# phlash/java-sdr

Hardware: AMD Instinct MI355X
Metric: IQ Msamples/s through FFT+FIR+BPSK demod, 2048-pt frames (higher is better)
Workload: dtype f64

## Files before the change

java-sdr_amd/csrc/bpsk_fm.hip:

```cpp
#include "bpsk_units.h"
#include "bpsk_tuner.h"
#include <math.h>
#include <type_traits>
#include <stddef.h>
#include <stdlib.h>

namespace jsdr {
namespace fm { __constant__ BpskConst c_bpsk; }
using fm::c_bpsk;
}
#include "bpsk_matched.h"

namespace jsdr {


template <bool FAST>
__global__ __launch_bounds__(512) void k_matched(MatchedArgs a)
{
    extern __shared__ __align__(16) unsigned char smem[];
    double2 *X = reinterpret_cast<double2 *>(smem);
    const int s = blockIdx.y;
    const long long G = a.tile0 + 4160LL * blockIdx.x;
    const double2 *dm = a.dm + (long long)s * a.dm_stride;
    {
// ... 69 lines not shown
__device__ unsigned long long g_fm_wgclk[WGCLK_SLOTS][WGCLK_WGS][3];
static long long g_wgclk_log[WGCLK_SLOTS][4];
#endif

__global__ void k_fm_edges(EdgeArgs a)
{
    const int t = blockIdx.x * blockDim.x + threadIdx.x;
    const int s = t / (4 * FM_EDGE), i = t % (4 * FM_EDGE);
    if (s >= a.nstreams) return;
    const int n = i < 2 * FM_EDGE ? i - FM_EDGE : a.nsamples - FM_EDGE + (i - 2 * FM_EDGE);
    int w = 0;
    if (n >= 0 && n < a.nsamples) {
        w = a.raw[(long long)s * a.stride_pairs + n];
    } else if (n < 0 && n >= -26) {
        w = a.hist[(long long)s * 32 + 26 + n].x;
        if (a.dc) {
            const int si = (int)(short)((w & 0xffff) - a.ic);
            const int sq = (int)(short)((w >> 16) - a.qc);
            w = (si & 0xffff) | (sq << 16);
        }
    }
    a.edges[(long long)s * (4 * FM_EDGE) + i] = w;
}

__global__ void k_fm_prep(EdgeArgs e, HistArgs hi, ScatterArgs sc)
{
    const int t = blockIdx.x * blockDim.x + threadIdx.x;
    const int nedge = e.nstreams * 4 * FM_EDGE;
    {
        const int v = t - nedge - 32 * e.nstreams;
        if (v >= 0) {
            if (v < sc.bytes[0]) sc.dst[0][v] = sc.src[0][v];
            else if (v - sc.bytes[0] < sc.bytes[1]) sc.dst[1][v - sc.bytes[0]] = sc.src[1][v - sc.bytes[0]];
            return;
        }
    }
    if (t < nedge) {
        const int s = t / (4 * FM_EDGE), i = t % (4 * FM_EDGE);
        const int n = i < 2 * FM_EDGE ? i - FM_EDGE : e.nsamples - FM_EDGE + (i - 2 * FM_EDGE);
        int w = 0;
        if (n >= 0 && n < e.nsamples) {
            w = e.raw[(long long)s * e.stride_pairs + n];
        } else if (n < 0 && n >= -26) {
            w = e.hist[(long long)s * 32 + 26 + n].x;
            if (e.dc) {
                const int si = (int)(short)((w & 0xffff) - e.ic);
                const int sq = (int)(short)((w >> 16) - e.qc);
                w = (si & 0xffff) | (sq << 16);
            }
        }
        e.edges[(long long)s * (4 * FM_EDGE) + i] = w;
        return;
    }
    const int u = t - nedge;
    const int s = u >> 5, i = u & 31;
    if (s >= hi.nstreams || i >= 26) return;
    const long long n = hi.nsamples - 26 + i;
    int2 v;
    if (n < 0) {
        v = hi.hist_old[(long long)s * 32 + (26 + n)];
    } else {
        const int w = hi.raw[(long long)s * hi.stride_pairs + n];
        const int si = java_short_add((int)(short)(w & 0xffff), hi.ic);
        const int sq = java_short_add(w >> 16, hi.qc);
        v = make_int2((si & 0xffff) | (sq << 16), 0);
    }
    hi.hist_new[(long long)s * 32 + i] = v;
}

constexpr bool ds_taps_are_short()
{
    for (int n = 0; n < 14; n++) {
        const float k = kDsHalf[n] * 32768.0f;
        if (k != (float)(int)k || k >= 16384.0f || k <= -16384.0f) return false;
    }
    return true;
}
static_assert(ds_taps_are_short(), "dsFilter: every tap times 2^15 is an integer of magnitude below 2^14 (k_fm's +-1.0 fmas are exact)");

template <int D, int R, bool MIX, bool DC, bool FAST, bool SMALL = false, int PH = -1>
#ifndef JSDR_FM_MINWAVES
#define JSDR_FM_MINWAVES 2
#endif
__global__ __launch_bounds__(FM_THREADS, JSDR_FM_MINWAVES) void k_fm(FmArgs a)
{
    constexpr int RD = D * R, NS = RD - D + 27, NSQ = (NS + 3) / 4;
    constexpr int JOBS = (FM_NT + R - 1) / R, ROUNDS = (JOBS + FM_THREADS - 1) / FM_THREADS;
    static_assert(PH < 0 || (MIX && !FAST && PH < 4 && (D * R) % 8 == 0 && (65 * FM_NB * D) % 8 == 4),
                  "k_fm<PH>: the lane span is whole periods and a tile is half a period past the one before");
    extern __shared__ __align__(16) unsigned char smem[];
    double2 *X = reinterpret_cast<double2 *>(smem);
    double *sc = reinterpret_cast<double *>(smem + FM_NT * sizeof(double2));
    for (int i = threadIdx.x; i < 512; i += FM_THREADS) sc[i] = a.sincos[i];
#ifdef JSDR_X_CLK
    unsigned long long clk_acc_[6] = {0, 0, 0, 0, 0, 0}, clk_last_ = 0;
#endif
#ifdef JSDR_X_WGCLK
    const unsigned long long wgclk0 = __builtin_amdgcn_s_memrealtime();
    unsigned long long wgclk_n = 0;
#endif
    const long long nwork = (long long)a.ntiles * a.nstreams;
    const bool tickets = a.tickets != nullptr;
    int *tkL = reinterpret_cast<int *>(sc + 512);
#pragma unroll 1
    for (long long work = blockIdx.x; work < nwork; work = tickets ? (long long)gridDim.x + (unsigned)__builtin_amdgcn_readfirstlane(tkL[0]) : work + gridDim.x) {
    const int s = (int)(work / a.ntiles);
    const long long G = a.tile0 + (long long)(65 * FM_NB) * (work % a.ntiles);
    const int jrel0 = (int)(G - 64 - a.g_first);
#ifdef JSDR_X_FM_SMALLSET
    const int *raw = a.raw + (long long)(s & 15) * a.stride_pairs;
#else
    const int *raw = a.raw + (long long)s * a.stride_pairs;
#endif
    const int *edges = a.edges + (long long)s * (4 * FM_EDGE);
    const double2 *dmh_old = a.dmh_old + (long long)s * 64;
    const int Lm1 = a.nsamples - 1, nds = a.nds, P = a.tper;
    const double HOWARD = 0.9 * 32768.0 * (double)I16_2P15_UNSCALE;
    int e0 = 0;
    if constexpr (MIX) {
        const long long v = (long long)a.first_out + (long long)D * jrel0;
        e0 = (int)(((v % P) + P) % P);
    }
    typedef const __attribute__((address_space(4))) double *const_tab_t;
    const_tab_t tb = (const_tab_t)(a.tcs + e0);
    float amx = 0.0f;
    __syncthreads();
#ifdef JSDR_X_CLK
    clk_last_ = __builtin_amdgcn_s_memtime();
#endif
    auto front = [&](auto phc) __attribute__((always_inline)) {
    constexpr int PHC = decltype(phc)::value;
#ifdef JSDR_X_NOFRONT
    if (a.nds < 0)
#endif
#pragma unroll 1
    for (int round = 0; round < ROUNDS; round++) {
        const int job = threadIdx.x + FM_THREADS * round;
        const int t0 = R * job;
        if (t0 >= FM_NT) break;
        const int j0 = jrel0 + t0;
        const int n0 = a.first_out + D * j0 - 26;
        const bool none = j0 + R <= 0 || j0 >= nds || nds <= 0;
        const bool regular = j0 >= 0 && j0 + R <= nds;
        if (!none) {
            int4 W[NSQ];
            const int *wp = raw + n0;
            if (n0 < 0) wp = edges + (n0 + FM_EDGE);
            else if (n0 + 4 * NSQ - 1 > Lm1) wp = edges + 2 * FM_EDGE + (n0 - (a.nsamples - FM_EDGE));
            unsigned kv4[(R + 3) / 4];
#pragma unroll
            for (int k = 0; k < (R + 3) / 4; k++) kv4[k] = 0;
            if (regular) {
#pragma unroll
                for (int r = 0; r < R; r++) kv4[r / 4] |= (unsigned)a.kvco[j0 + r] << (8 * (r % 4));
            } else {
#pragma unroll
                for (int r = 0; r < R; r++) {
                    const int j = j0 + r;
                    kv4[r / 4] |= (unsigned)a.kvco[j < 0 ? 0 : (j >= nds ? nds - 1 : j)] << (8 * (r % 4));
                }
            }
#pragma unroll
            for (int q = NSQ - 1; q >= 0; q--) W[q] = *reinterpret_cast<const int4 *>(wp + 4 * q);
#ifndef JSDR_FM_NOPIN
            __builtin_amdgcn_sched_barrier(0);
#endif
            double ai[R], aq[R];
            double vc[R], vs[R];
#pragma unroll
            for (int r = 0; r < R; r++) {
                ai[r] = 0.0;
                aq[r] = 0.0;
            }
#pragma unroll
            for (int q = NSQ - 1; q >= 0; q--) {
                const int4 w4 = W[q];
                if (q == 0) {
#pragma unroll
                    for (int r = 0; r < R; r++) {
                        const int kv = (kv4[r / 4] >> (8 * (r % 4))) & 0xff;
                        vc[r] = sc[kv];
                        vs[r] = sc[256 + kv];
                    }
                }
#pragma unroll
                for (int t = 3; t >= 0; t--) {
                    const int m = 4 * q + t;
                    if (m < NS) {
                        const int w = (t == 0) ? w4.x : (t == 1) ? w4.y : (t == 2) ? w4.z : w4.w;
                        double di, dq;
                        fm_convert_2p15(w, a.ic, a.qc, DC, di, dq, FAST ? &amx : nullptr);
                        const int ci = PHC >= 0 ? tuner8_class(PHC + m, 0) : TC_GEN, cq = PHC >= 0 ? tuner8_class(PHC + m, 1) : TC_GEN;
                        if constexpr (MIX) {
                            if (ci == TC_GEN) di = di * tb[2 * m];
                            if (cq == TC_GEN) dq = dq * tb[2 * m + 1];
                        }
#pragma unroll
                        for (int r = 0; r < R; r++) {
                            if (m >= D * r && m <= D * r + 26) {
                                const int age = D * r + 26 - m;
                                const double tp = ds_tap(age);
                                const bool same = age == 0 || ((kDsPow2Mask >> age) & 1);
                                if (FAST || same || ci != TC_GEN) {
                                    if (ci != TC_ZERO) ai[r] = __builtin_fma(di, ci == TC_MONE ? -tp : tp, ai[r]);
                                } else {
                                    ai[r] += di * tp;
                                }
                                if (FAST || same || cq != TC_GEN) {
                                    if (cq != TC_ZERO) aq[r] = __builtin_fma(dq, cq == TC_MONE ? -tp : tp, aq[r]);
                                } else {
                                    aq[r] += dq * tp;
                                }
                            }
                        }
                    }
                }
#ifndef JSDR_FM_NOPIN
#pragma unroll
                for (int r = 0; r < R; r++) asm volatile("" : "+v"(ai[r]), "+v"(aq[r])::"memory");
                if constexpr (FAST) asm volatile("" : "+v"(amx));
                __builtin_amdgcn_sched_barrier(0);
#endif
            }
            if (regular) {
#pragma unroll
                for (int r = 0; r < R; r++) {
                    const double oi = ai[r] * HOWARD, oq = aq[r] * HOWARD;
                    if (FM_NT % R == 0 || t0 + r < FM_NT) X[t0 + r] = make_double2(oi * vc[r], oq * vs[r]);
                }
            } else {
                double oi[R], oq[R];
#pragma unroll
                for (int r = 0; r < R; r++) {
                    oi[r] = ai[r] * HOWARD * vc[r];
                    oq[r] = aq[r] * HOWARD * vs[r];
                }
#pragma unroll 1
                for (int r = 0; r < R; r++) {
                    const int t = t0 + r, j = j0 + r;
                    double2 val = make_double2(0.0, 0.0);
                    if (j >= 0 && j < nds) {
                        val.x = r == 0 ? oi[0] : r == 1 ? oi[1] : r == 2 ? oi[2] : r == 3 ? oi[3] : oi[R - 1];
                        val.y = r == 0 ? oq[0] : r == 1 ? oq[1] : r == 2 ? oq[2] : r == 3 ? oq[3] : oq[R - 1];
                    } else if (j >= -64 && j < 0) {
                        val = dmh_old[64 + j];
                    }
                    if (t < FM_NT) X[t] = val;
                }
            }
        } else {
#pragma unroll 1
            for (int r = 0; r < R; r++) {
                const int t = t0 + r, j = j0 + r;
                const double2 val = (j >= -64 && j < 0) ? dmh_old[64 + j] : make_double2(0.0, 0.0);
                if (t < FM_NT) X[t] = val;
            }
        }
    }
    };
    if constexpr (PH < 0) {
        front(std::integral_constant<int, -1>{});
    } else {
        if (((e0 + a.trot) & 7) == PH) front(std::integral_constant<int, PH>{});
        else front(std::integral_constant<int, PH + 4>{});
    }
    if constexpr (FAST) {
#pragma unroll
        for (int off = 32; off >= 1; off >>= 1) amx = fmaxf(amx, __shfl_xor(amx, off, 64));
        if ((threadIdx.x & 63) == 0 && amx > 0.0f) atomicMax(a.amax + s, __float_as_int(amx));
    }
    FM_CLK(1);
    __syncthreads();
    FM_CLK(3);
    unsigned tk = 0;
    if (tickets && threadIdx.x == 0) tk = atomicAdd(a.tickets, 1u);
    if (jrel0 + FM_NT > nds - 64) {
        double2 *dmh_new = a.dmh_new + (long long)s * 64;
        for (int t = 64 + threadIdx.x; t < FM_NT; t += FM_THREADS) {
            const int j = jrel0 + t;
            if (j >= nds - 64 && j < nds && j >= 0) dmh_new[j - (nds - 64)] = X[t];
        }
        if (work % a.ntiles == 0 && nds < 64 && (int)threadIdx.x < 64 - nds) dmh_new[threadIdx.x] = dmh_old[threadIdx.x + nds];
    }
    const int lane = threadIdx.x & 63;
    const int wave = __builtin_amdgcn_readfirstlane(threadIdx.x >> 6);
    const int blk = lane < FM_NB ? lane : FM_NB - 1;
    const double2 *xl = X + 64 + 65 * blk;
    const int rel0 = jrel0 + 64 + 65 * blk;
    double2 *y = a.y + (long long)s * a.y_stride;
    if constexpr (SMALL) {
        const int rel = (int)threadIdx.x, t = rel - jrel0;
        if (rel < nds && t >= 64 && t < FM_NT) {
            const long long g = a.g_first + rel;
            const int u = (int)(((g - 64) % 65 + 65) % 65);
            const double2 *xg = X + t;
            const double *f = c_bpsk.dm_taps;
            double yi = 0.0, yq = 0.0;
            for (int i = 0; i <= 64 - u; i++) {
                const double2 x = xg[-(u + i)];
                const double tp = f[u + i];
                if constexpr (FAST) {
                    yi = __builtin_fma(x.x, tp, yi);
                    yq = __builtin_fma(x.y, tp, yq);
                } else {
                    yi += x.x * tp;
                    yq += x.y * tp;
                }
            }
            for (int m = 0; m < u; m++) {
                const double2 x = xg[-m];
                const double tp = f[m];
                if constexpr (FAST) {
                    yi = __builtin_fma(x.x, tp, yi);
                    yq = __builtin_fma(x.y, tp, yq);
                } else {
                    yi += x.x * tp;
                    yq += x.y * tp;
                }
            }
            y[rel] = make_double2(yi, yq);
        }
    } else {
#ifdef JSDR_X_NOMATCHED
    if (a.nds < 0)
#endif
#ifndef JSDR_FM_DIRECT_STORE
    {
        double ai[9], aq[9];
        int u0 = 0, nout = 9;
        if (wave == 0) {
            matched_block<9, FAST>(xl, 0, ai, aq);
        } else {
            u0 = 9 + 8 * (wave - 1);
            nout = 8;
            double bi[8], bq[8];
            matched_block<8, FAST>(xl, u0, bi, bq);
#pragma unroll
            for (int r = 0; r < 8; r++) {
                ai[r] = bi[r];
                aq[r] = bq[r];
            }
        }
        __syncthreads();
        if (lane < FM_NB) {
#pragma unroll
            for (int r = 0; r < 9; r++)
                if (r < nout) X[65 * blk + u0 + r] = make_double2(ai[r], aq[r]);
        }
        __syncthreads();
        const int relb = jrel0 + 64;
        for (int o = (int)threadIdx.x; o < 65 * FM_NB; o += FM_THREADS) {
            const int rel = relb + o;
            if (rel >= 0 && rel < nds) y[rel] = X[o];
        }
    }
#else
    if (wave == 0) {
        double ai[9], aq[9];
        matched_block<9, FAST>(xl, 0, ai, aq);
#pragma unroll
        for (int r = 0; r < 9; r++) {
            const int rel = rel0 + r;
            if (lane < FM_NB && rel >= 0 && rel < nds) y[rel] = make_double2(ai[r], aq[r]);
        }
    } else {
        const int u0 = 9 + 8 * (wave - 1);
        double ai[8], aq[8];
        matched_block<8, FAST>(xl, u0, ai, aq);
#pragma unroll
        for (int r = 0; r < 8; r++) {
            const int rel = rel0 + u0 + r;
            if (lane < FM_NB && rel >= 0 && rel < nds) y[rel] = make_double2(ai[r], aq[r]);
        }
    }
#endif
    }
    FM_CLK(4);
    {
        int zlate = 0;
        asm volatile("" : "+v"(zlate));
        if (tickets && threadIdx.x == 0) tkL[0] = (int)tk + zlate;
    }
    __syncthreads();
    FM_CLK(5);
#ifdef JSDR_X_WGCLK
    wgclk_n++;
#endif
    }
#ifdef JSDR_X_WGCLK
    if (threadIdx.x == 0 && blockIdx.x < WGCLK_WGS) {
        unsigned long long *c = g_fm_wgclk[a.wgclk_slot][blockIdx.x];
        c[0] = wgclk0;
        c[1] = __builtin_amdgcn_s_memrealtime();
        c[2] = wgclk_n;
    }
#endif
#ifdef JSDR_X_CLK
    if ((threadIdx.x & 63) == 0)
        for (int i = 0; i < 6; i++) atomicAdd(&g_fm_clk[blockIdx.x & 255][(threadIdx.x >> 6) * 8 + i], clk_acc_[i]);
#endif
}


int bpsk_fm_upload_constants(const BpskConst &bc)
{
    JSDR_HIP_TRY(hipMemcpyToSymbol(HIP_SYMBOL(c_bpsk), &bc, sizeof(bc)));
    return JSDR_OK;
}

int launch_matched(const MatchedArgs &ma, int nstreams, hipStream_t st)
{
    const long long ntiles = (ma.g_first + ma.nds - ma.tile0 + 4159) / 4160;
    const size_t lds = (64 + 4160) * sizeof(double2);
    JSDR_LDS_ATTR(k_matched<false>, lds);
    JSDR_LDS_ATTR(k_matched<true>, lds);
    hipLaunchKernelGGL(k_matched<false>, dim3((unsigned)ntiles, (unsigned)nstreams), dim3(512), lds, st, ma);
    return launched();
}

int launch_dm_history(double2 *dm, long long dm_stride, long long nds, int nstreams, hipStream_t st)
{
    hipLaunchKernelGGL(k_dm_history, dim3((unsigned)nstreams), dim3(64), 0, st, dm, dm_stride, nds, nstreams);
    return launched();
}

int launch_fm_prep(const EdgeArgs &ea, const HistArgs &ha, const ScatterArgs &sc, hipStream_t st)
{
    hipLaunchKernelGGL(k_fm_prep, dim3((unsigned)(((long long)ea.nstreams * (4 * FM_EDGE + 32) + sc.bytes[0] + sc.bytes[1] + 255) / 256)),
                       dim3(256), 0, st, ea, ha, sc);
    return launched();
}

template <int D, int R>
static int launch_fm_t(const FmArgs &a_in, bool mix, bool dc, bool fast, int nstreams, hipStream_t st, long long *items, long long *grid_out,
                       int *phase)
{
    *phase = -1;
    const size_t lds = (size_t)FM_NT * sizeof(double2) + 512 * sizeof(double) + sizeof(double);
    const long long span = 65LL * FM_NB;
    const long long ntiles = (a_in.g_first + a_in.nds - a_in.tile0 + span - 1) / span;
    FmArgs a = a_in;
    a.ntiles = (int)ntiles;
    a.nstreams = nstreams;
    static const long long grid_cap = [] {
        const char *e = knob("JSDR_FM_GRID");
        return e ? atoll(e) : 0LL;
    }();
    long long gx = ntiles * nstreams;
    if (grid_cap > 0 && gx > grid_cap) gx = grid_cap;
    if (a.grid_limit > 0 && gx > a.grid_limit) gx = a.grid_limit;
    *items = ntiles * nstreams;
    *grid_out = gx;
    if (!(a.grid_limit > 0 && gx < ntiles * nstreams && ntiles * nstreams + gx < 0x7fffffffLL)) a.tickets = nullptr;
#ifdef JSDR_X_WGCLK
    {
        static int wgclk_seq = 0;
        static const bool wgclk_static = getenv("JSDR_X_WGCLK_STATIC") != nullptr;
        if (wgclk_static) a.tickets = nullptr;
        a.wgclk_slot = wgclk_seq % WGCLK_SLOTS;
        g_wgclk_log[a.wgclk_slot][0] = ntiles * nstreams;
        g_wgclk_log[a.wgclk_slot][1] = gx;
        g_wgclk_log[a.wgclk_slot][2] = a.tickets != nullptr;
        g_wgclk_log[a.wgclk_slot][3] = wgclk_seq++;
    }
#endif
    if (a.tickets) JSDR_HIP_TRY(hipMemsetAsync(a.tickets, 0, sizeof(unsigned), st));
    const dim3 grid((unsigned)gx), block(FM_THREADS);
#define JSDR_FM_LAUNCH_PH(MIX, DC, FAST, SMALL, PH)                                                             \
    do {                                                                                                        \
        JSDR_LDS_ATTR((k_fm<D, R, MIX, DC, FAST, SMALL, PH>), lds);                                             \
        hipLaunchKernelGGL((k_fm<D, R, MIX, DC, FAST, SMALL, PH>), grid, block, lds, st, a);                    \
    } while (0)
#define JSDR_FM_LAUNCH(MIX, DC, FAST, SMALL) JSDR_FM_LAUNCH_PH(MIX, DC, FAST, SMALL, -1)
    const bool small = !fast && a.nds <= FM_THREADS && ntiles == 1;
    if constexpr (D == 10) {
        if (mix && !fast && !small && a.trot >= 0 && a.tper == 8) {
            const long long v = (long long)a.first_out + (long long)D * (a.tile0 - 64 - a.g_first);
            const int p0 = (int)((((v % 8) + 8) % 8 + a.trot) & 7);
            *phase = p0;
            switch (p0 & 3) {
                case 0: if (dc) JSDR_FM_LAUNCH_PH(true, true, false, false, 0); else JSDR_FM_LAUNCH_PH(true, false, false, false, 0); break;
                case 1: if (dc) JSDR_FM_LAUNCH_PH(true, true, false, false, 1); else JSDR_FM_LAUNCH_PH(true, false, false, false, 1); break;
                case 2: if (dc) JSDR_FM_LAUNCH_PH(true, true, false, false, 2); else JSDR_FM_LAUNCH_PH(true, false, false, false, 2); break;
                default: if (dc) JSDR_FM_LAUNCH_PH(true, true, false, false, 3); else JSDR_FM_LAUNCH_PH(true, false, false, false, 3); break;
// ... 76 lines not shown
```

java-sdr_amd/csrc/bpsk_fm_f32.hip:

```cpp
#include "bpsk_units.h"
#include <math.h>
#include <stddef.h>
#include <stdlib.h>

namespace jsdr {
namespace fm32 { __constant__ BpskConst c_bpsk; }
using fm32::c_bpsk;
}
#include "bpsk_matched.h"

namespace jsdr {

#ifndef JSDR_FM32_PQ
#define JSDR_FM32_PQ 6
#endif
enum { FM32_PQ = JSDR_FM32_PQ };

__global__ void k_fm_prep_f32(EdgeF32Args e, HistArgs hi)
{
    const int t = blockIdx.x * blockDim.x + threadIdx.x;
    const int nedge = e.nstreams * 4 * FM_EDGE;
    if (t < nedge) {
        const int s = t / (4 * FM_EDGE), i = t % (4 * FM_EDGE);
        const int n = i < 2 * FM_EDGE ? i - FM_EDGE : e.nsamples - FM_EDGE + (i - 2 * FM_EDGE);
        float2 w = make_float2(0.0f, 0.0f);
        if (n >= 0 && n < e.nsamples) {
            w = e.rawf[(long long)s * e.stride_pairs + n];
        } else if (n < 0 && n >= -26) {
            const int2 h = e.hist[(long long)s * 32 + 26 + n];
            w = make_float2(__int_as_float(h.x), __int_as_float(h.y));
        }
        e.edges[(long long)s * (4 * FM_EDGE) + i] = w;
        return;
    }
    const int u = t - nedge;
    const int s = u >> 5, i = u & 31;
    if (s >= hi.nstreams || i >= 26) return;
    const long long n = hi.nsamples - 26 + i;
    int2 v;
    if (n < 0) {
        v = hi.hist_old[(long long)s * 32 + (26 + n)];
    } else {
        const float2 f = hi.rawf[(long long)s * hi.stride_pairs + n];
        v = make_int2(__float_as_int(f.x), __float_as_int(f.y));
    }
    hi.hist_new[(long long)s * 32 + i] = v;
}

template <int D, int R, bool MIX, bool SMALL = false>
__global__ __launch_bounds__(FM_THREADS, 2) void k_fm_f32(FmF32Args fa)
{
    const FmArgs &a = fa.a;
    constexpr int RD = D * R, NS = RD - D + 27, NQ = (NS + 1) / 2;
    constexpr int PQ = FM32_PQ, NP = (NQ + PQ - 1) / PQ;
    constexpr int JOBS = (FM_NT + R - 1) / R, ROUNDS = (JOBS + FM_THREADS - 1) / FM_THREADS;
    static_assert(2 * NQ <= FM_EDGE, "a window must fit an edge image's half");
    extern __shared__ __align__(16) unsigned char smem[];
    double2 *X = reinterpret_cast<double2 *>(smem);
    double *sc = reinterpret_cast<double *>(smem + FM_NT * sizeof(double2));
    for (int i = threadIdx.x; i < 512; i += FM_THREADS) sc[i] = a.sincos[i];
    const long long nwork = (long long)a.ntiles * a.nstreams;
    const bool tickets = a.tickets != nullptr;
    int *tkL = reinterpret_cast<int *>(sc + 512);
#pragma unroll 1
    for (long long work = blockIdx.x; work < nwork; work = tickets ? (long long)gridDim.x + (unsigned)__builtin_amdgcn_readfirstlane(tkL[0]) : work + gridDim.x) {
    const int s = (int)(work / a.ntiles);
    const long long G = a.tile0 + (long long)(65 * FM_NB) * (work % a.ntiles);
    const int jrel0 = (int)(G - 64 - a.g_first);
    const float2 *raw = fa.rawf + (long long)s * a.stride_pairs;
    const float2 *edges = fa.edges + (long long)s * (4 * FM_EDGE);
    const double2 *dmh_old = a.dmh_old + (long long)s * 64;
    const int Lm1 = a.nsamples - 1, nds = a.nds, P = a.tper;
    const double HOWARD = 0.9 * 32768.0;
    int e0 = 0;
    if constexpr (MIX) {
        const long long v = (long long)a.first_out + (long long)D * jrel0;
        e0 = (int)(((v % P) + P) % P);
    }
    typedef const __attribute__((address_space(4))) double *const_tab_t;
    const_tab_t tb = (const_tab_t)(a.tcs + e0);
    __syncthreads();
#pragma unroll 1
    for (int round = 0; round < ROUNDS; round++) {
        const int job = threadIdx.x + FM_THREADS * round;
        const int t0 = R * job;
        if (t0 >= FM_NT) break;
        const int j0 = jrel0 + t0;
        const int n0 = a.first_out + D * j0 - 26;
        const bool none = j0 + R <= 0 || j0 >= nds || nds <= 0;
        const bool regular = j0 >= 0 && j0 + R <= nds;
        if (!none) {
            const float2 *wp = raw + n0;
            if (n0 < 0) wp = edges + (n0 + FM_EDGE);
            else if (n0 + 2 * NQ - 1 > Lm1) wp = edges + 2 * FM_EDGE + (n0 - (a.nsamples - FM_EDGE));
            unsigned kv4[(R + 3) / 4];
#pragma unroll
            for (int k = 0; k < (R + 3) / 4; k++) kv4[k] = 0;
            if (regular) {
#pragma unroll
                for (int r = 0; r < R; r++) kv4[r / 4] |= (unsigned)a.kvco[j0 + r] << (8 * (r % 4));
            } else {
#pragma unroll
                for (int r = 0; r < R; r++) {
                    const int j = j0 + r;
                    kv4[r / 4] |= (unsigned)a.kvco[j < 0 ? 0 : (j >= nds ? nds - 1 : j)] << (8 * (r % 4));
                }
            }
            float4 W[2][PQ];
#pragma unroll
            for (int p = 0; p < 2 && p < NP; p++) {
#pragma unroll
                for (int k = 0; k < PQ; k++) {
                    const int q = NQ - 1 - PQ * p - k;
                    if (q >= 0) W[p][k] = *reinterpret_cast<const float4 *>(wp + 2 * q);
                }
            }
            __builtin_amdgcn_sched_barrier(0);
            double ai[R], aq[R];
            double vc[R], vs[R];
#pragma unroll
            for (int r = 0; r < R; r++) {
                ai[r] = 0.0;
                aq[r] = 0.0;
            }
#pragma unroll
            for (int p = 0; p < NP; p++) {
#pragma unroll
                for (int k = 0; k < PQ; k++) {
                    const int q = NQ - 1 - PQ * p - k;
                    if (q >= 0) {
                        const float4 w4 = W[p & 1][k];
                        if (q == 0) {
#pragma unroll
                            for (int r = 0; r < R; r++) {
                                const int kv = (kv4[r / 4] >> (8 * (r % 4))) & 0xff;
                                vc[r] = sc[kv];
                                vs[r] = sc[256 + kv];
                            }
                        }
#pragma unroll
                        for (int t = 1; t >= 0; t--) {
                            const int m = 2 * q + t;
                            if (m < NS) {
                                double di = (double)(t ? w4.z : w4.x);
                                double dq = (double)(t ? w4.w : w4.y);
                                if constexpr (MIX) {
                                    di = di * tb[2 * m];
                                    dq = dq * tb[2 * m + 1];
                                }
#pragma unroll
                                for (int r = 0; r < R; r++) {
                                    if (m >= D * r && m <= D * r + 26) {
                                        const double tp = ds_tap(D * r + 26 - m);
                                        ai[r] += di * tp;
                                        aq[r] += dq * tp;
                                    }
                                }
                            }
                        }
                        if ((k & 1) || q == 0) {
#pragma unroll
                            for (int r = 0; r < R; r++) asm volatile("" : "+v"(ai[r]), "+v"(aq[r])::"memory");
                            __builtin_amdgcn_sched_barrier(0);
                        }
                    }
                }
                if (p + 2 < NP) {
#pragma unroll
                    for (int k = 0; k < PQ; k++) {
                        const int q = NQ - 1 - PQ * (p + 2) - k;
                        if (q >= 0) W[p & 1][k] = *reinterpret_cast<const float4 *>(wp + 2 * q);
                    }
                    __builtin_amdgcn_sched_barrier(0);
                }
            }
            if (regular) {
#pragma unroll
                for (int r = 0; r < R; r++) {
                    const double oi = ai[r] * HOWARD, oq = aq[r] * HOWARD;
                    if (FM_NT % R == 0 || t0 + r < FM_NT) X[t0 + r] = make_double2(oi * vc[r], oq * vs[r]);
                }
            } else {
                double oi[R], oq[R];
#pragma unroll
                for (int r = 0; r < R; r++) {
                    oi[r] = ai[r] * HOWARD * vc[r];
                    oq[r] = aq[r] * HOWARD * vs[r];
                }
#pragma unroll 1
                for (int r = 0; r < R; r++) {
                    const int t = t0 + r, j = j0 + r;
                    double2 val = make_double2(0.0, 0.0);
                    if (j >= 0 && j < nds) {
                        val.x = r == 0 ? oi[0] : r == 1 ? oi[1] : r == 2 ? oi[2] : r == 3 ? oi[3] : oi[R - 1];
                        val.y = r == 0 ? oq[0] : r == 1 ? oq[1] : r == 2 ? oq[2] : r == 3 ? oq[3] : oq[R - 1];
                    } else if (j >= -64 && j < 0) {
                        val = dmh_old[64 + j];
                    }
                    if (t < FM_NT) X[t] = val;
                }
            }
        } else {
#pragma unroll 1
            for (int r = 0; r < R; r++) {
                const int t = t0 + r, j = j0 + r;
                const double2 val = (j >= -64 && j < 0) ? dmh_old[64 + j] : make_double2(0.0, 0.0);
                if (t < FM_NT) X[t] = val;
            }
        }
    }
    __syncthreads();
    unsigned tk = 0;
    if (tickets && threadIdx.x == 0) tk = atomicAdd(a.tickets, 1u);
    if (jrel0 + FM_NT > nds - 64) {
        double2 *dmh_new = a.dmh_new + (long long)s * 64;
        for (int t = 64 + threadIdx.x; t < FM_NT; t += FM_THREADS) {
            const int j = jrel0 + t;
            if (j >= nds - 64 && j < nds && j >= 0) dmh_new[j - (nds - 64)] = X[t];
        }
        if (work % a.ntiles == 0 && nds < 64 && (int)threadIdx.x < 64 - nds) dmh_new[threadIdx.x] = dmh_old[threadIdx.x + nds];
    }
    const int lane = threadIdx.x & 63;
    const int wave = __builtin_amdgcn_readfirstlane(threadIdx.x >> 6);
    const int blk = lane < FM_NB ? lane : FM_NB - 1;
    const double2 *xl = X + 64 + 65 * blk;
    double2 *y = a.y + (long long)s * a.y_stride;
    if constexpr (SMALL) {
        const int rel = (int)threadIdx.x, t = rel - jrel0;
        if (rel < nds && t >= 64 && t < FM_NT) {
            const long long g = a.g_first + rel;
            const int u = (int)(((g - 64) % 65 + 65) % 65);
            const double2 *xg = X + t;
            const double *f = c_bpsk.dm_taps;
            double yi = 0.0, yq = 0.0;
            for (int i = 0; i <= 64 - u; i++) {
                const double2 x = xg[-(u + i)];
                const double tp = f[u + i];
                yi += x.x * tp;
                yq += x.y * tp;
            }
            for (int m = 0; m < u; m++) {
                const double2 x = xg[-m];
                const double tp = f[m];
                yi += x.x * tp;
                yq += x.y * tp;
            }
            y[rel] = make_double2(yi, yq);
        }
    } else {
        double ai[9], aq[9];
        int u0 = 0, nout = 9;
        if (wave == 0) {
            matched_block<9, false>(xl, 0, ai, aq);
        } else {
            u0 = 9 + 8 * (wave - 1);
            nout = 8;
            double bi[8], bq[8];
            matched_block<8, false>(xl, u0, bi, bq);
#pragma unroll
            for (int r = 0; r < 8; r++) {
                ai[r] = bi[r];
                aq[r] = bq[r];
            }
        }
        __syncthreads();
        if (lane < FM_NB) {
#pragma unroll
            for (int r = 0; r < 9; r++)
                if (r < nout) X[65 * blk + u0 + r] = make_double2(ai[r], aq[r]);
        }
        __syncthreads();
        const int relb = jrel0 + 64;
        for (int o = (int)threadIdx.x; o < 65 * FM_NB; o += FM_THREADS) {
            const int rel = relb + o;
            if (rel >= 0 && rel < nds) y[rel] = X[o];
        }
    }
    {
        int zlate = 0;
        asm volatile("" : "+v"(zlate));
        if (tickets && threadIdx.x == 0) tkL[0] = (int)tk + zlate;
    }
    __syncthreads();
    }
}

int bpsk_fm_f32_upload_constants(const BpskConst &bc)
{
    JSDR_HIP_TRY(hipMemcpyToSymbol(HIP_SYMBOL(c_bpsk), &bc, sizeof(bc)));
    return JSDR_OK;
}

int launch_fm_prep_f32(const EdgeF32Args &ea, const HistArgs &ha, hipStream_t st)
{
    hipLaunchKernelGGL(k_fm_prep_f32, dim3((unsigned)(((long long)ea.nstreams * (4 * FM_EDGE + 32) + 255) / 256)), dim3(256), 0, st, ea, ha);
    return launched();
}

template <int D, int R>
static int launch_fm_f32_t(const FmF32Args &a_in, bool mix, int nstreams, hipStream_t st, long long *items, long long *grid_out)
{
    const size_t lds = (size_t)FM_NT * sizeof(double2) + 512 * sizeof(double) + sizeof(double);
    const long long span = 65LL * FM_NB;
    const long long ntiles = (a_in.a.g_first + a_in.a.nds - a_in.a.tile0 + span - 1) / span;
    FmF32Args a = a_in;
    a.a.ntiles = (int)ntiles;
    a.a.nstreams = nstreams;
    long long gx = ntiles * nstreams;
    if (a.a.grid_limit > 0 && gx > a.a.grid_limit) gx = a.a.grid_limit;
    *items = ntiles * nstreams;
    *grid_out = gx;
    if (!(a.a.grid_limit > 0 && gx < ntiles * nstreams && ntiles * nstreams + gx < 0x7fffffffLL)) a.a.tickets = nullptr;
    if (a.a.tickets) JSDR_HIP_TRY(hipMemsetAsync(a.a.tickets, 0, sizeof(unsigned), st));
    const dim3 grid((unsigned)gx), block(FM_THREADS);
#define JSDR_FM32_LAUNCH(MIX, SMALL)                                              \
    do {                                                                          \
        JSDR_LDS_ATTR((k_fm_f32<D, R, MIX, SMALL>), lds);                         \
        hipLaunchKernelGGL((k_fm_f32<D, R, MIX, SMALL>), grid, block, lds, st, a); \
    } while (0)
    if (a.a.nds <= FM_THREADS && ntiles == 1) {
        if (mix) JSDR_FM32_LAUNCH(true, true); else JSDR_FM32_LAUNCH(false, true);
    } else {
        if (mix) JSDR_FM32_LAUNCH(true, false); else JSDR_FM32_LAUNCH(false, false);
    }
#undef JSDR_FM32_LAUNCH
    return launched();
}

int launch_fm_f32(const FmF32Args &a, int decim, bool mix, int nstreams, hipStream_t st, long long *items, long long *grid)
{
    switch (decim) {
        case 4: return launch_fm_f32_t<4, 5>(a, mix, nstreams, st, items, grid);
        case 5: return launch_fm_f32_t<5, 4>(a, mix, nstreams, st, items, grid);
        case 10: return launch_fm_f32_t<10, 4>(a, mix, nstreams, st, items, grid);
        case 20: return launch_fm_f32_t<20, 4>(a, mix, nstreams, st, items, grid);
    }
    set_error("bpsk: unsupported decimation %d", decim);
    return JSDR_ERR;
}

}
```

java-sdr_amd/csrc/bpsk_matched.h:

```cpp
#pragma once

namespace jsdr {


template <int R, bool FAST = false>
__device__ __forceinline__ void matched_block(const double2 *xl , int u0, double (&ai)[R],
                                              double (&aq)[R])
{
    const double *f = c_bpsk.dm_taps;
    const int n1 = 66 - u0 - R;
    {
        const double2 v = xl[0];
#pragma unroll
        for (int r = 0; r < R; r++) {
            const double t = f[u0 + r];
            ai[r] = __builtin_fma(v.x, t, 0.0);
            aq[r] = __builtin_fma(v.y, t, 0.0);
        }
    }
    int i = 1;
#ifndef JSDR_MATCHED_NO_CHUNKS
    for (; i + 8 <= n1; i += 8) {
        double tw[8 + R - 1];
#pragma unroll
        for (int k = 0; k < 8 + R - 1; k++) tw[k] = f[u0 + i + k];
        double2 v8[8];
#pragma unroll
        for (int k = 0; k < 8; k++) v8[k] = xl[-(i + k)];
#pragma unroll
        for (int k = 0; k < 8; k++) {
#pragma unroll
            for (int r = 0; r < R; r++) {
                if constexpr (FAST) {
                    ai[r] = __builtin_fma(v8[k].x, tw[k + r], ai[r]);
                    aq[r] = __builtin_fma(v8[k].y, tw[k + r], aq[r]);
                } else {
                    ai[r] += v8[k].x * tw[k + r];
                    aq[r] += v8[k].y * tw[k + r];
                }
            }
        }
    }
#endif
    for (; i < n1; i++) {
        double2 v = xl[-i];
#pragma unroll
        for (int r = 0; r < R; r++) {
            double t = f[u0 + i + r];
            if constexpr (FAST) {
                ai[r] = __builtin_fma(v.x, t, ai[r]);
                aq[r] = __builtin_fma(v.y, t, aq[r]);
            } else {
                ai[r] += v.x * t;
                aq[r] += v.y * t;
            }
        }
    }
#pragma unroll
    for (int q = 0; q < R - 1; q++) {
        const int i2 = n1 + q;
        double2 v = xl[-i2];
#pragma unroll
        for (int r = 0; r < R - 1 - q; r++) {
            double t = f[u0 + i2 + r];
            if constexpr (FAST) {
                ai[r] = __builtin_fma(v.x, t, ai[r]);
                aq[r] = __builtin_fma(v.y, t, aq[r]);
            } else {
                ai[r] += v.x * t;
                aq[r] += v.y * t;
            }
        }
    }
#pragma unroll
    for (int q = 0; q < R - 1; q++) {
        double2 v = xl[u0 + R - 1 - q];
#pragma unroll
        for (int r = R - 1 - q; r < R; r++) {
            double t = f[r - (R - 1 - q)];
            if constexpr (FAST) {
                ai[r] = __builtin_fma(v.x, t, ai[r]);
                aq[r] = __builtin_fma(v.y, t, aq[r]);
            } else {
                ai[r] += v.x * t;
                aq[r] += v.y * t;
            }
        }
    }
    int m = 0;
#ifndef JSDR_MATCHED_NO_CHUNKS
    for (; m + 8 <= u0; m += 8) {
        double tw[8 + R - 1];
#pragma unroll
        for (int k = 0; k < 8 + R - 1; k++) tw[k] = f[m + k];
        double2 v8[8];
#pragma unroll
        for (int k = 0; k < 8; k++) v8[k] = xl[u0 - (m + k)];
#pragma unroll
        for (int k = 0; k < 8; k++) {
#pragma unroll
            for (int r = 0; r < R; r++) {
                if constexpr (FAST) {
                    ai[r] = __builtin_fma(v8[k].x, tw[k + r], ai[r]);
                    aq[r] = __builtin_fma(v8[k].y, tw[k + r], aq[r]);
                } else {
                    ai[r] += v8[k].x * tw[k + r];
                    aq[r] += v8[k].y * tw[k + r];
                }
            }
        }
    }
#endif
    for (; m < u0; m++) {
        double2 v = xl[u0 - m];
#pragma unroll
        for (int r = 0; r < R; r++) {
            double t = f[r + m];
            if constexpr (FAST) {
                ai[r] = __builtin_fma(v.x, t, ai[r]);
                aq[r] = __builtin_fma(v.y, t, aq[r]);
            } else {
                ai[r] += v.x * t;
                aq[r] += v.y * t;
            }
        }
    }
}

}
```

java-sdr_amd/csrc/common.h:

```cpp
#pragma once
#include <hip/hip_runtime.h>
#include <stdint.h>
#include <stdio.h>
#include <stdlib.h>
#include <string.h>
#include <atomic>
#include <string>
#include <type_traits>
#include <utility>
#include "../../include/jsdr_hip.h"

namespace jsdr {

void set_error(const char *fmt, ...);

#define JSDR_HIP_TRY(expr)                                                                         \
    do {                                                                                           \
        hipError_t _e = (expr);                                                                    \
        if (_e != hipSuccess) {                                                                    \
            ::jsdr::set_error("%s failed: %s (%s:%d)", #expr, hipGetErrorString(_e), __FILE__,     \
                              __LINE__);                                                           \
            (void)hipGetLastError();   \
            return JSDR_ERR;                                                                       \
        }                                                                                          \
// ... 153 lines not shown
            live_pinned++;
        } else {
            (void)hipGetLastError();
        }
        return p != nullptr;
    }
    void release()
    {
        if (p) {
            (void)hipHostFree(p);
            live_pinned--;
        }
        p = nullptr;
        bytes = 0;
    }
};
using PinnedStage = Pinned<unsigned char>;

static_assert(!std::is_copy_constructible<DevBuf<int>>::value && std::is_nothrow_move_constructible<DevBuf<int>>::value, "DevBuf is move-only");
static_assert(!std::is_copy_constructible<Stream>::value && std::is_nothrow_move_constructible<Stream>::value, "Stream is move-only");
static_assert(!std::is_copy_constructible<Event>::value && std::is_nothrow_move_constructible<Event>::value, "Event is move-only");
static_assert(!std::is_copy_constructible<PinnedStage>::value && std::is_nothrow_move_constructible<PinnedStage>::value, "PinnedStage is move-only");

struct SyncOnExit {
    bool armed = true;
    ~SyncOnExit()
    {
        if (armed) (void)hipDeviceSynchronize();
    }
};

__device__ __forceinline__ float i16_to_float_java(int s)
{
    const float rh = 0x1.0002p-15f;
    const float rl = 0x1.0002p-45f;
    const float a = (float)s;
    return __builtin_fmaf(a, rh, a * rl);
}

constexpr float I16_2P15_UNSCALE = 0x1p-15f;
__device__ __forceinline__ float i16_to_float_java_2p15(int s)
{
    const float a = (float)s;
    return __builtin_fmaf(a, 0x1.0002p-15f, a);
}

__device__ __forceinline__ int java_short_add(int s, int corr)
{
    return (int)(short)(s + (int)(short)corr);
}

__device__ __forceinline__ void fm_convert(int w, int ic, int qc, bool dc, double &di, double &dq, float *amax = nullptr)
{
    int si = (int)(short)(w & 0xffff), sq = w >> 16;
    if (dc) {
        si = java_short_add(si, ic);
        sq = java_short_add(sq, qc);
    }
    typedef float v2f __attribute__((ext_vector_type(2)));
    const v2f a = {(float)si, (float)sq};
    if (amax) *amax = fmaxf(fmaxf(fabsf(a.x), fabsf(a.y)), *amax);
    const v2f rh = {0x1.0002p-15f, 0x1.0002p-15f}, rl = {0x1.0002p-45f, 0x1.0002p-45f};
    const v2f q = __builtin_elementwise_fma(a, rh, a * rl);
    di = (double)q.x;
    dq = (double)q.y;
}

__device__ __forceinline__ void fm_convert_2p15(int w, int ic, int qc, bool dc, double &di, double &dq, float *amax = nullptr)
{
    int si = (int)(short)(w & 0xffff), sq = w >> 16;
    if (dc) {
        si = java_short_add(si, ic);
        sq = java_short_add(sq, qc);
    }
    typedef float v2f __attribute__((ext_vector_type(2)));
    const v2f a = {(float)si, (float)sq};
    if (amax) *amax = fmaxf(fmaxf(fabsf(a.x), fabsf(a.y)), *amax);
    const v2f c = {0x1.0002p-15f, 0x1.0002p-15f};
    const v2f q = __builtin_elementwise_fma(a, c, a);
    di = (double)q.x;
    dq = (double)q.y;
}

}
```

Baseline: 247,100.

## Reload kernel args from kernarg segment at use sites and add short-tile matched path

Reads FmArgs through the kernarg segment pointer at each use site, with an asm barrier so the fields are re-fetched as scalar loads instead of being held live across the kernel. This is meant to cut register pressure. It also switches the work/tile split to 32-bit unsigned division when that is safe, and skips converting the unused rail when the tuner class for I or Q is zero. A new single-output matched-filter path handles short tiles where every output fits in one thread. The cost is extra scalar loads, plus a second, less-unrolled matched-filter loop on partial tiles.

```diff
diff --git a/java-sdr_amd/csrc/bpsk_fm.hip b/java-sdr_amd/csrc/bpsk_fm.hip
--- a/java-sdr_amd/csrc/bpsk_fm.hip
+++ b/java-sdr_amd/csrc/bpsk_fm.hip
@@ -175,12 +175,20 @@
 #ifndef JSDR_FM_MINWAVES
 #define JSDR_FM_MINWAVES 2
 #endif
-__global__ __launch_bounds__(FM_THREADS, JSDR_FM_MINWAVES) void k_fm(FmArgs a)
+__global__ __launch_bounds__(FM_THREADS, JSDR_FM_MINWAVES) void k_fm(FmArgs a_kernarg)
 {
     constexpr int RD = D * R, NS = RD - D + 27, NSQ = (NS + 3) / 4;
     constexpr int JOBS = (FM_NT + R - 1) / R, ROUNDS = (JOBS + FM_THREADS - 1) / FM_THREADS;
     static_assert(PH < 0 || (MIX && !FAST && PH < 4 && (D * R) % 8 == 0 && (65 * FM_NB * D) % 8 == 4),
                   "k_fm<PH>: the lane span is whole periods and a tile is half a period past the one before");
+    (void)a_kernarg;
+    typedef const __attribute__((address_space(4))) FmArgs *fm_args_t;
+    fm_args_t ap = (fm_args_t)__builtin_amdgcn_kernarg_segment_ptr();
+#define FM_ARGS_HERE                    \
+    fm_args_t ap_here = ap;             \
+    asm volatile("" : "+s"(ap_here));   \
+    const auto &a = *ap_here
+    FM_ARGS_HERE;
     extern __shared__ __align__(16) unsigned char smem[];
     double2 *X = reinterpret_cast<double2 *>(smem);
     double *sc = reinterpret_cast<double *>(smem + FM_NT * sizeof(double2));
@@ -197,25 +205,35 @@
     int *tkL = reinterpret_cast<int *>(sc + 512);
 #pragma unroll 1
     for (long long work = blockIdx.x; work < nwork; work = tickets ? (long long)gridDim.x + (unsigned)__builtin_amdgcn_readfirstlane(tkL[0]) : work + gridDim.x) {
-    const int s = (int)(work / a.ntiles);
-    const long long G = a.tile0 + (long long)(65 * FM_NB) * (work % a.ntiles);
-    const int jrel0 = (int)(G - 64 - a.g_first);
-#ifdef JSDR_X_FM_SMALLSET
-    const int *raw = a.raw + (long long)(s & 15) * a.stride_pairs;
-#else
-    const int *raw = a.raw + (long long)s * a.stride_pairs;
-#endif
-    const int *edges = a.edges + (long long)s * (4 * FM_EDGE);
-    const double2 *dmh_old = a.dmh_old + (long long)s * 64;
-    const int Lm1 = a.nsamples - 1, nds = a.nds, P = a.tper;
+    int s, tile, jrel0, nds;
+    {
+        FM_ARGS_HERE;
+        if (nwork <= 0x7fffffffLL) {
+            s = (int)((unsigned)work / (unsigned)a.ntiles);
+            tile = (int)((unsigned)work % (unsigned)a.ntiles);
+        } else {
+            s = (int)(work / a.ntiles);
+            tile = (int)(work % a.ntiles);
+        }
+        const long long G = a.tile0 + (long long)(65 * FM_NB) * tile;
+        jrel0 = (int)(G - 64 - a.g_first);
+        nds = a.nds;
+    }
     const double HOWARD = 0.9 * 32768.0 * (double)I16_2P15_UNSCALE;
     int e0 = 0;
+    bool ph_lo = true;
     if constexpr (MIX) {
+        FM_ARGS_HERE;
         const long long v = (long long)a.first_out + (long long)D * jrel0;
-        e0 = (int)(((v % P) + P) % P);
+        if constexpr (PH >= 0) {
+            e0 = (int)(v & 7);
+            ph_lo = ((e0 + a.trot) & 7) == PH;
+        } else {
+            const int P = a.tper;
+            e0 = (int)(((v % P) + P) % P);
+        }
     }
     typedef const __attribute__((address_space(4))) double *const_tab_t;
-    const_tab_t tb = (const_tab_t)(a.tcs + e0);
     float amx = 0.0f;
     __syncthreads();
 #ifdef JSDR_X_CLK
@@ -224,13 +242,22 @@
     auto front = [&](auto phc) __attribute__((always_inline)) {
     constexpr int PHC = decltype(phc)::value;
 #ifdef JSDR_X_NOFRONT
-    if (a.nds < 0)
+    if (nds < 0)
 #endif
 #pragma unroll 1
     for (int round = 0; round < ROUNDS; round++) {
         const int job = threadIdx.x + FM_THREADS * round;
         const int t0 = R * job;
         if (t0 >= FM_NT) break;
+        FM_ARGS_HERE;
+#ifdef JSDR_X_FM_SMALLSET
+        const int *raw = a.raw + (long long)(s & 15) * a.stride_pairs;
+#else
+        const int *raw = a.raw + (long long)s * a.stride_pairs;
+#endif
+        const int *edges = a.edges + (long long)s * (4 * FM_EDGE);
+        const int Lm1 = a.nsamples - 1;
+        const_tab_t tb = (const_tab_t)(a.tcs + e0);
         const int j0 = jrel0 + t0;
         const int n0 = a.first_out + D * j0 - 26;
         const bool none = j0 + R <= 0 || j0 >= nds || nds <= 0;
@@ -281,9 +308,17 @@
                     const int m = 4 * q + t;
                     if (m < NS) {
                         const int w = (t == 0) ? w4.x : (t == 1) ? w4.y : (t == 2) ? w4.z : w4.w;
+                        const int ci = PHC >= 0 ? tuner8_class(PHC + m, 0) : TC_GEN, cq = PHC >= 0 ? tuner8_class(PHC + m, 1) : TC_GEN;
                         double di, dq;
-                        fm_convert_2p15(w, a.ic, a.qc, DC, di, dq, FAST ? &amx : nullptr);
-                        const int ci = PHC >= 0 ? tuner8_class(PHC + m, 0) : TC_GEN, cq = PHC >= 0 ? tuner8_class(PHC + m, 1) : TC_GEN;
+                        if (!FAST && cq == TC_ZERO && ci != TC_ZERO) {
+                            di = fm_convert_2p15_rail((int)(short)(w & 0xffff), a.ic, DC);
+                            dq = 0.0;
+                        } else if (!FAST && ci == TC_ZERO && cq != TC_ZERO) {
+                            di = 0.0;
+                            dq = fm_convert_2p15_rail(w >> 16, a.qc, DC);
+                        } else {
+                            fm_convert_2p15(w, a.ic, a.qc, DC, di, dq, FAST ? &amx : nullptr);
+                        }
                         if constexpr (MIX) {
                             if (ci == TC_GEN) di = di * tb[2 * m];
                             if (cq == TC_GEN) dq = dq * tb[2 * m + 1];
@@ -336,7 +371,7 @@
                         val.x = r == 0 ? oi[0] : r == 1 ? oi[1] : r == 2 ? oi[2] : r == 3 ? oi[3] : oi[R - 1];
                         val.y = r == 0 ? oq[0] : r == 1 ? oq[1] : r == 2 ? oq[2] : r == 3 ? oq[3] : oq[R - 1];
                     } else if (j >= -64 && j < 0) {
-                        val = dmh_old[64 + j];
+                        val = a.dmh_old[(long long)s * 64 + 64 + j];
                     }
                     if (t < FM_NT) X[t] = val;
                 }
@@ -345,7 +380,7 @@
 #pragma unroll 1
             for (int r = 0; r < R; r++) {
                 const int t = t0 + r, j = j0 + r;
-                const double2 val = (j >= -64 && j < 0) ? dmh_old[64 + j] : make_double2(0.0, 0.0);
+                const double2 val = (j >= -64 && j < 0) ? a.dmh_old[(long long)s * 64 + 64 + j] : make_double2(0.0, 0.0);
                 if (t < FM_NT) X[t] = val;
             }
         }
@@ -354,36 +389,42 @@
     if constexpr (PH < 0) {
         front(std::integral_constant<int, -1>{});
     } else {
-        if (((e0 + a.trot) & 7) == PH) front(std::integral_constant<int, PH>{});
+        if (ph_lo) front(std::integral_constant<int, PH>{});
         else front(std::integral_constant<int, PH + 4>{});
     }
     if constexpr (FAST) {
 #pragma unroll
         for (int off = 32; off >= 1; off >>= 1) amx = fmaxf(amx, __shfl_xor(amx, off, 64));
+        FM_ARGS_HERE;
         if ((threadIdx.x & 63) == 0 && amx > 0.0f) atomicMax(a.amax + s, __float_as_int(amx));
     }
     FM_CLK(1);
     __syncthreads();
     FM_CLK(3);
     unsigned tk = 0;
-    if (tickets && threadIdx.x == 0) tk = atomicAdd(a.tickets, 1u);
+    {
+        FM_ARGS_HERE;
+        if (tickets && threadIdx.x == 0) tk = atomicAdd(a.tickets, 1u);
+    }
     if (jrel0 + FM_NT > nds - 64) {
+        FM_ARGS_HERE;
         double2 *dmh_new = a.dmh_new + (long long)s * 64;
         for (int t = 64 + threadIdx.x; t < FM_NT; t += FM_THREADS) {
             const int j = jrel0 + t;
             if (j >= nds - 64 && j < nds && j >= 0) dmh_new[j - (nds - 64)] = X[t];
         }
-        if (work % a.ntiles == 0 && nds < 64 && (int)threadIdx.x < 64 - nds) dmh_new[threadIdx.x] = dmh_old[threadIdx.x + nds];
+        if (tile == 0 && nds < 64 && (int)threadIdx.x < 64 - nds) dmh_new[threadIdx.x] = a.dmh_old[(long long)s * 64 + threadIdx.x + nds];
     }
     const int lane = threadIdx.x & 63;
     const int wave = __builtin_amdgcn_readfirstlane(threadIdx.x >> 6);
     const int blk = lane < FM_NB ? lane : FM_NB - 1;
     const double2 *xl = X + 64 + 65 * blk;
-    const int rel0 = jrel0 + 64 + 65 * blk;
-    double2 *y = a.y + (long long)s * a.y_stride;
+    [[maybe_unused]] const dm_taps_t taps = dm_taps_here();
     if constexpr (SMALL) {
         const int rel = (int)threadIdx.x, t = rel - jrel0;
         if (rel < nds && t >= 64 && t < FM_NT) {
+            FM_ARGS_HERE;
+            double2 *y = a.y + (long long)s * a.y_stride;
             const long long g = a.g_first + rel;
             const int u = (int)(((g - 64) % 65 + 65) % 65);
             const double2 *xg = X + t;
@@ -414,20 +455,31 @@
             y[rel] = make_double2(yi, yq);
         }
     } else {
+#ifndef JSDR_FM_NO_SHORT_TILE
+    const int olo = jrel0 + 64 > 0 ? jrel0 + 64 : 0, ohi = jrel0 + FM_NT < nds ? jrel0 + FM_NT : nds;
+    if (ohi - olo <= FM_THREADS) {
+        const int rel = olo + (int)threadIdx.x, t = rel - jrel0;
+        if (rel < ohi) {
+            const double2 v = matched_single<FAST>(X + t, (t - 64) % 65);
+            FM_ARGS_HERE;
+            (a.y + (long long)s * a.y_stride)[rel] = v;
+        }
+    } else
+#endif
 #ifdef JSDR_X_NOMATCHED
-    if (a.nds < 0)
+    if (nds < 0)
 #endif
 #ifndef JSDR_FM_DIRECT_STORE
     {
         double ai[9], aq[9];
         int u0 = 0, nout = 9;
         if (wave == 0) {
-            matched_block<9, FAST>(xl, 0, ai, aq);
+            matched_block<9, FAST>(xl, 0, ai, aq, taps);
         } else {
             u0 = 9 + 8 * (wave - 1);
             nout = 8;
             double bi[8], bq[8];
-            matched_block<8, FAST>(xl, u0, bi, bq);
+            matched_block<8, FAST>(xl, u0, bi, bq, taps);
 #pragma unroll
             for (int r = 0; r < 8; r++) {
                 ai[r] = bi[r];
@@ -441,6 +493,8 @@
                 if (r < nout) X[65 * blk + u0 + r] = make_double2(ai[r], aq[r]);
         }
         __syncthreads();
+        FM_ARGS_HERE;
+        double2 *y = a.y + (long long)s * a.y_stride;
         const int relb = jrel0 + 64;
         for (int o = (int)threadIdx.x; o < 65 * FM_NB; o += FM_THREADS) {
             const int rel = relb + o;
@@ -449,8 +503,11 @@
     }
 #else
     if (wave == 0) {
+        const int rel0 = jrel0 + 64 + 65 * blk;
         double ai[9], aq[9];
-        matched_block<9, FAST>(xl, 0, ai, aq);
+        matched_block<9, FAST>(xl, 0, ai, aq, taps);
+        FM_ARGS_HERE;
+        double2 *y = a.y + (long long)s * a.y_stride;
 #pragma unroll
         for (int r = 0; r < 9; r++) {
             const int rel = rel0 + r;
@@ -458,8 +515,11 @@
         }
     } else {
         const int u0 = 9 + 8 * (wave - 1);
+        const int rel0 = jrel0 + 64 + 65 * blk;
         double ai[8], aq[8];
-        matched_block<8, FAST>(xl, u0, ai, aq);
+        matched_block<8, FAST>(xl, u0, ai, aq, taps);
+        FM_ARGS_HERE;
+        double2 *y = a.y + (long long)s * a.y_stride;
 #pragma unroll
         for (int r = 0; r < 8; r++) {
             const int rel = rel0 + u0 + r;
@@ -493,6 +553,7 @@
         for (int i = 0; i < 6; i++) atomicAdd(&g_fm_clk[blockIdx.x & 255][(threadIdx.x >> 6) * 8 + i], clk_acc_[i]);
 #endif
 }
+#undef FM_ARGS_HERE
 
 
 int bpsk_fm_upload_constants(const BpskConst &bc)
diff --git a/java-sdr_amd/csrc/bpsk_fm_f32.hip b/java-sdr_amd/csrc/bpsk_fm_f32.hip
--- a/java-sdr_amd/csrc/bpsk_fm_f32.hip
+++ b/java-sdr_amd/csrc/bpsk_fm_f32.hip
@@ -48,9 +48,17 @@
 }
 
 template <int D, int R, bool MIX, bool SMALL = false>
-__global__ __launch_bounds__(FM_THREADS, 2) void k_fm_f32(FmF32Args fa)
-{
-    const FmArgs &a = fa.a;
+__global__ __launch_bounds__(FM_THREADS, 2) void k_fm_f32(FmF32Args fa_kernarg)
+{
+    (void)fa_kernarg;
+    typedef const __attribute__((address_space(4))) FmF32Args *fm_args_t;
+    const fm_args_t ap = (fm_args_t)__builtin_amdgcn_kernarg_segment_ptr();
+#define FM32_ARGS_HERE                  \
+    fm_args_t ap_here = ap;             \
+    asm volatile("" : "+s"(ap_here));   \
+    const auto &fa = *ap_here;          \
+    const auto &a = fa.a
+    FM32_ARGS_HERE;
     constexpr int RD = D * R, NS = RD - D + 27, NQ = (NS + 1) / 2;
     constexpr int PQ = FM32_PQ, NP = (NQ + PQ - 1) / PQ;
     constexpr int JOBS = (FM_NT + R - 1) / R, ROUNDS = (JOBS + FM_THREADS - 1) / FM_THREADS;
@@ -64,27 +72,39 @@
     int *tkL = reinterpret_cast<int *>(sc + 512);
 #pragma unroll 1
     for (long long work = blockIdx.x; work < nwork; work = tickets ? (long long)gridDim.x + (unsigned)__builtin_amdgcn_readfirstlane(tkL[0]) : work + gridDim.x) {
-    const int s = (int)(work / a.ntiles);
-    const long long G = a.tile0 + (long long)(65 * FM_NB) * (work % a.ntiles);
-    const int jrel0 = (int)(G - 64 - a.g_first);
-    const float2 *raw = fa.rawf + (long long)s * a.stride_pairs;
-    const float2 *edges = fa.edges + (long long)s * (4 * FM_EDGE);
-    const double2 *dmh_old = a.dmh_old + (long long)s * 64;
-    const int Lm1 = a.nsamples - 1, nds = a.nds, P = a.tper;
+    int s, tile, jrel0, nds, e0 = 0;
+    {
+        FM32_ARGS_HERE;
+        (void)fa;
+        if (nwork <= 0x7fffffffLL) {
+            s = (int)((unsigned)work / (unsigned)a.ntiles);
+            tile = (int)((unsigned)work % (unsigned)a.ntiles);
+        } else {
+            s = (int)(work / a.ntiles);
+            tile = (int)(work % a.ntiles);
+        }
+        const long long G = a.tile0 + (long long)(65 * FM_NB) * tile;
+        jrel0 = (int)(G - 64 - a.g_first);
+        nds = a.nds;
+        if constexpr (MIX) {
+            const int P = a.tper;
+            const long long v = (long long)a.first_out + (long long)D * jrel0;
+            e0 = (int)(((v % P) + P) % P);
+        }
+    }
     const double HOWARD = 0.9 * 32768.0;
-    int e0 = 0;
-    if constexpr (MIX) {
-        const long long v = (long long)a.first_out + (long long)D * jrel0;
-        e0 = (int)(((v % P) + P) % P);
-    }
     typedef const __attribute__((address_space(4))) double *const_tab_t;
-    const_tab_t tb = (const_tab_t)(a.tcs + e0);
     __syncthreads();
 #pragma unroll 1
     for (int round = 0; round < ROUNDS; round++) {
         const int job = threadIdx.x + FM_THREADS * round;
         const int t0 = R * job;
         if (t0 >= FM_NT) break;
+        FM32_ARGS_HERE;
+        const float2 *raw = fa.rawf + (long long)s * a.stride_pairs;
+        const float2 *edges = fa.edges + (long long)s * (4 * FM_EDGE);
+        const int Lm1 = a.nsamples - 1;
+        [[maybe_unused]] const_tab_t tb = (const_tab_t)(a.tcs + e0);
         const int j0 = jrel0 + t0;
         const int n0 = a.first_out + D * j0 - 26;
         const bool none = j0 + R <= 0 || j0 >= nds || nds <= 0;
@@ -195,7 +215,7 @@
                         val.x = r == 0 ? oi[0] : r == 1 ? oi[1] : r == 2 ? oi[2] : r == 3 ? oi[3] : oi[R - 1];
                         val.y = r == 0 ? oq[0] : r == 1 ? oq[1] : r == 2 ? oq[2] : r == 3 ? oq[3] : oq[R - 1];
                     } else if (j >= -64 && j < 0) {
-                        val = dmh_old[64 + j];
+                        val = a.dmh_old[(long long)s * 64 + 64 + j];
                     }
                     if (t < FM_NT) X[t] = val;
                 }
@@ -204,30 +224,39 @@
 #pragma unroll 1
             for (int r = 0; r < R; r++) {
                 const int t = t0 + r, j = j0 + r;
-                const double2 val = (j >= -64 && j < 0) ? dmh_old[64 + j] : make_double2(0.0, 0.0);
+                const double2 val = (j >= -64 && j < 0) ? a.dmh_old[(long long)s * 64 + 64 + j] : make_double2(0.0, 0.0);
                 if (t < FM_NT) X[t] = val;
             }
         }
     }
     __syncthreads();
     unsigned tk = 0;
-    if (tickets && threadIdx.x == 0) tk = atomicAdd(a.tickets, 1u);
+    {
+        FM32_ARGS_HERE;
+        (void)fa;
+        if (tickets && threadIdx.x == 0) tk = atomicAdd(a.tickets, 1u);
+    }
     if (jrel0 + FM_NT > nds - 64) {
+        FM32_ARGS_HERE;
+        (void)fa;
         double2 *dmh_new = a.dmh_new + (long long)s * 64;
         for (int t = 64 + threadIdx.x; t < FM_NT; t += FM_THREADS) {
             const int j = jrel0 + t;
             if (j >= nds - 64 && j < nds && j >= 0) dmh_new[j - (nds - 64)] = X[t];
         }
-        if (work % a.ntiles == 0 && nds < 64 && (int)threadIdx.x < 64 - nds) dmh_new[threadIdx.x] = dmh_old[threadIdx.x + nds];
+        if (tile == 0 && nds < 64 && (int)threadIdx.x < 64 - nds) dmh_new[threadIdx.x] = a.dmh_old[(long long)s * 64 + threadIdx.x + nds];
     }
     const int lane = threadIdx.x & 63;
     const int wave = __builtin_amdgcn_readfirstlane(threadIdx.x >> 6);
     const int blk = lane < FM_NB ? lane : FM_NB - 1;
     const double2 *xl = X + 64 + 65 * blk;
-    double2 *y = a.y + (long long)s * a.y_stride;
+    [[maybe_unused]] const dm_taps_t taps = dm_taps_here();
     if constexpr (SMALL) {
         const int rel = (int)threadIdx.x, t = rel - jrel0;
         if (rel < nds && t >= 64 && t < FM_NT) {
+            FM32_ARGS_HERE;
+            (void)fa;
+            double2 *y = a.y + (long long)s * a.y_stride;
             const long long g = a.g_first + rel;
             const int u = (int)(((g - 64) % 65 + 65) % 65);
             const double2 *xg = X + t;
@@ -247,16 +276,24 @@
             }
             y[rel] = make_double2(yi, yq);
         }
+    } else if (const int olo = jrel0 + 64 > 0 ? jrel0 + 64 : 0, ohi = jrel0 + FM_NT < nds ? jrel0 + FM_NT : nds; ohi - olo <= FM_THREADS) {
+        const int rel = olo + (int)threadIdx.x, t = rel - jrel0;
+        if (rel < ohi) {
+            const double2 v = matched_single<false>(X + t, (t - 64) % 65);
+            FM32_ARGS_HERE;
+            (void)fa;
+            (a.y + (long long)s * a.y_stride)[rel] = v;
+        }
     } else {
         double ai[9], aq[9];
         int u0 = 0, nout = 9;
         if (wave == 0) {
-            matched_block<9, false>(xl, 0, ai, aq);
+            matched_block<9, false>(xl, 0, ai, aq, taps);
         } else {
             u0 = 9 + 8 * (wave - 1);
             nout = 8;
             double bi[8], bq[8];
-            matched_block<8, false>(xl, u0, bi, bq);
+            matched_block<8, false>(xl, u0, bi, bq, taps);
 #pragma unroll
             for (int r = 0; r < 8; r++) {
                 ai[r] = bi[r];
@@ -270,6 +307,9 @@
                 if (r < nout) X[65 * blk + u0 + r] = make_double2(ai[r], aq[r]);
         }
         __syncthreads();
+        FM32_ARGS_HERE;
+        (void)fa;
+        double2 *y = a.y + (long long)s * a.y_stride;
         const int relb = jrel0 + 64;
         for (int o = (int)threadIdx.x; o < 65 * FM_NB; o += FM_THREADS) {
             const int rel = relb + o;
@@ -284,6 +324,7 @@
     __syncthreads();
     }
 }
+#undef FM32_ARGS_HERE
 
 int bpsk_fm_f32_upload_constants(const BpskConst &bc)
 {
diff --git a/java-sdr_amd/csrc/bpsk_matched.h b/java-sdr_amd/csrc/bpsk_matched.h
--- a/java-sdr_amd/csrc/bpsk_matched.h
+++ b/java-sdr_amd/csrc/bpsk_matched.h
@@ -3,11 +3,18 @@
 namespace jsdr {
 
 
+typedef const __attribute__((address_space(4))) double *dm_taps_t;
+__device__ __forceinline__ dm_taps_t dm_taps_here()
+{
+    dm_taps_t f = (dm_taps_t)c_bpsk.dm_taps;
+    asm volatile("" : "+s"(f));
+    return f;
+}
+
 template <int R, bool FAST = false>
 __device__ __forceinline__ void matched_block(const double2 *xl , int u0, double (&ai)[R],
-                                              double (&aq)[R])
+                                              double (&aq)[R], dm_taps_t f = (dm_taps_t)c_bpsk.dm_taps)
 {
-    const double *f = c_bpsk.dm_taps;
     const int n1 = 66 - u0 - R;
     {
         const double2 v = xl[0];
@@ -127,4 +134,34 @@
     }
 }
 
+template <bool FAST = false>
+__device__ __forceinline__ double2 matched_single(const double2 *xg , int u )
+{
+    const double *f = c_bpsk.dm_taps;
+    double yi = 0.0, yq = 0.0;
+    for (int i = 0; i <= 64 - u; i++) {
+        const double2 x = xg[-(u + i)];
+        const double tp = f[u + i];
+        if constexpr (FAST) {
+            yi = __builtin_fma(x.x, tp, yi);
+            yq = __builtin_fma(x.y, tp, yq);
+        } else {
+            yi += x.x * tp;
+            yq += x.y * tp;
+        }
+    }
+    for (int m = 0; m < u; m++) {
+        const double2 x = xg[-m];
+        const double tp = f[m];
+        if constexpr (FAST) {
+            yi = __builtin_fma(x.x, tp, yi);
+            yq = __builtin_fma(x.y, tp, yq);
+        } else {
+            yi += x.x * tp;
+            yq += x.y * tp;
+        }
+    }
+    return make_double2(yi, yq);
 }
+
+}
diff --git a/java-sdr_amd/csrc/common.h b/java-sdr_amd/csrc/common.h
--- a/java-sdr_amd/csrc/common.h
+++ b/java-sdr_amd/csrc/common.h
@@ -259,4 +259,11 @@
     dq = (double)q.y;
 }
 
-}
+__device__ __forceinline__ double fm_convert_2p15_rail(int s, int c, bool dc)
+{
+    if (dc) s = java_short_add(s, c);
+    const float a = (float)s;
+    return (double)__builtin_fmaf(a, 0x1.0002p-15f, a);
+}
+
+}
```

Measured after the change: 250,600, median of 6. 1.4% higher.
